# dash-robotics/perception

Measured on AMD Instinct MI355X. Metric: frames/sec (640x480 D435 cloud, plane+cluster+ICP), higher is better.
Workload: dtype f32

## Files before the change

### perception_amd/csrc/k_icp_lat.hip

```cpp
#include "kernels.hpp"
#include "icp_solve.hpp"

namespace cd {

struct LatFaces {
    int nface;
    unsigned m0[LAT_MAX_FACES], m1[LAT_MAX_FACES], m2[LAT_MAX_FACES];
    float c[LAT_MAX_FACES];
    int nx, ny, nz, tox, toy, toz;
    float ox, oy, oz, ivx, ivy, ivz;
};

template <int THREADS>
__device__ __forceinline__ void lat_stage(const IcpLattice* __restrict__ L, LatFaces& F, float4* s_tab, int4* s_face) {
    F.nface = L->nface;
#pragma unroll
    for (int f = 0; f < LAT_MAX_FACES; ++f) { F.m0[f] = L->m0[f]; F.m1[f] = L->m1[f]; F.m2[f] = L->m2[f]; F.c[f] = L->c[f]; }
    F.nx = L->n[0]; F.ny = L->n[1]; F.nz = L->n[2]; F.tox = L->toff[0]; F.toy = L->toff[1]; F.toz = L->toff[2];
    F.ox = L->noi[0]; F.oy = L->noi[1]; F.oz = L->noi[2]; F.ivx = L->inv[0]; F.ivy = L->inv[1]; F.ivz = L->inv[2];
    for (int i = threadIdx.x; i < L->ntab; i += THREADS) s_tab[i] = L->tab[i];
    if (threadIdx.x < LAT_MAX_FACES) {
        const int f = threadIdx.x, w = L->w[f], u = L->fast[f], v = 3 - w - u;
        s_face[f] = make_int4(w, u, L->base[f], __float_as_int(L->c[f]));
        s_face[LAT_MAX_FACES + f] = make_int4(L->toff[u], L->toff[v < 0 || v > 2 ? 0 : v], L->n[u], 0);
    }
    __syncthreads();
}

__device__ __forceinline__ float lat_pick(unsigned m, float a, float b) {
    float r;
    asm("v_bfi_b32 %0, %1, %2, %3" : "=v"(r) : "s"(m), "v"(a), "v"(b));
    return r;
}

__device__ __forceinline__ void lat_axis(const float4* s_tab, int toff, int n, float o_inv_neg, float inv, float q, float& f, int& ig_out, bool& lo_out,
                                         bool& hi_out, float& t, float& gap) {
    int ig;
    {
        const float pos = __builtin_fmaf(q, inv, o_inv_neg);
        asm("v_cvt_rpi_i32_f32 %0, %1" : "=v"(ig) : "v"(pos));
    }
    ig = min(max(ig, 0), n - 1);
    const float4 W = s_tab[toff + ig];
    const float d0 = __fsub_rn(q, W.x), d1 = __fsub_rn(q, W.y), d2 = __fsub_rn(q, W.z);
    const float f0 = __fmul_rn(d0, d0), f1 = __fmul_rn(d1, d1), f2 = __fmul_rn(d2, d2);
    const float g_mid = __fsub_rn(f0, f1), g_hi = __fsub_rn(f1, f2);
    const bool lo = f0 < f1;
    const bool hi = f2 < f1;
    f = f1; t = W.y; gap = g_mid;
    f = lo ? f0 : f; t = lo ? W.x : t; gap = lo ? 0.f : gap;
    f = hi ? f2 : f; t = hi ? W.z : t; gap = hi ? g_hi : gap;
    ig_out = ig; lo_out = lo; hi_out = hi;
}

__device__ __forceinline__ float lat_sum(float ax, float ay, float az) { return __fadd_rn(__fadd_rn(ax, ay), az); }

struct LatHit {
    float d;
    float nx, ny, nz;
    int face;
    int ix, iy, iz;
};

template <bool TIES, int NF>
__device__ __forceinline__ LatHit lat_nearest(const float4* s_tab, const int4* s_face, const LatFaces& F, float qx, float qy, float qz) {
    float fx, fy, fz, tx, ty, tz, gx, gy, gz;
    int cx, cy, cz;
    bool lox, hix, loy, hiy, loz, hiz;
    LatHit h;
    lat_axis(s_tab, F.tox, F.nx, F.ox, F.ivx, qx, fx, cx, lox, hix, tx, gx);
    lat_axis(s_tab, F.toy, F.ny, F.oy, F.ivy, qy, fy, cy, loy, hiy, ty, gy);
    lat_axis(s_tab, F.toz, F.nz, F.oz, F.ivz, qz, fz, cz, loz, hiz, tz, gz);
    h.ix = h.iy = h.iz = 0;
    h.d = __uint_as_float(0x7f800000u); h.face = 0;
#pragma unroll
    for (int f = 0; f < NF; ++f) {
        const unsigned m0 = F.m0[f], m1 = F.m1[f], m2 = F.m2[f];
        const float dc = __fsub_rn(lat_pick(m0, qx, lat_pick(m1, qy, qz)), F.c[f]);
        const float fc = __fmul_rn(dc, dc);
        const float d = lat_sum(lat_pick(m0, fc, fx), lat_pick(m1, fc, fy), lat_pick(m2, fc, fz));
        const bool better = d < h.d;
        h.d = better ? d : h.d;
        if (TIES) h.face = better ? f : h.face;
    }
    h.nx = tx; h.ny = ty; h.nz = tz;
    if (TIES) {
        const int4 fd = s_face[h.face];
        const float c = __int_as_float(fd.w);
        h.nx = fd.x == 0 ? c : tx; h.ny = fd.x == 1 ? c : ty; h.nz = fd.x == 2 ? c : tz;
        const float gsel = fd.x == 0 ? fminf(gy, gz) : (fd.x == 1 ? fminf(gx, gz) : fminf(gx, gy));
        const bool maybe = gsel <= __fmul_rn(h.d, 4.76837158203125e-07f);
        if (ballot64(maybe)) {
            h.ix = cx + (hix ? 1 : 0) - (lox ? 1 : 0); h.iy = cy + (hiy ? 1 : 0) - (loy ? 1 : 0); h.iz = cz + (hiz ? 1 : 0) - (loz ? 1 : 0);
            for (int f = 0; f < F.nface; ++f) {
                const bool mine = maybe && h.face == f;
                if (!ballot64(mine)) continue;
                const int4 gd = s_face[f];
                const int w = __builtin_amdgcn_readfirstlane(gd.x), u = __builtin_amdgcn_readfirstlane(gd.y), v = 3 - w - u;
                const float cc = __int_as_float(__builtin_amdgcn_readfirstlane(gd.w));
                const int4 ge = s_face[LAT_MAX_FACES + f];
                const int toff_u = __builtin_amdgcn_readfirstlane(ge.x), toff_v = __builtin_amdgcn_readfirstlane(ge.y);
                const float qw = w == 0 ? qx : (w == 1 ? qy : qz), qu = u == 0 ? qx : (u == 1 ? qy : qz), qv = v == 0 ? qx : (v == 1 ? qy : qz);
                const float dc = __fsub_rn(qw, cc);
                const float fc = __fmul_rn(dc, dc);
                float fu = u == 0 ? fx : (u == 1 ? fy : fz), fv = v == 0 ? fx : (v == 1 ? fy : fz);
                float tu = u == 0 ? tx : (u == 1 ? ty : tz), tv = v == 0 ? tx : (v == 1 ? ty : tz);
                int iu = u == 0 ? h.ix : (u == 1 ? h.iy : h.iz), iv = v == 0 ? h.ix : (v == 1 ? h.iy : h.iz);
                auto d_of = [&](float a_u, float a_v) {
                    const float ax = w == 0 ? fc : (u == 0 ? a_u : a_v), ay = w == 1 ? fc : (u == 1 ? a_u : a_v), az = w == 2 ? fc : (u == 2 ? a_u : a_v);
                    return lat_sum(ax, ay, az);
                };
                for (;;) {
                    const int j = max(iv - 1, 0);
                    const float t = s_tab[toff_v + j].y;
                    const float dd = __fsub_rn(qv, t);
                    const float a = __fmul_rn(dd, dd);
                    const bool go = mine && iv > 0 && d_of(fu, a) == h.d;
                    iv = go ? j : iv; fv = go ? a : fv; tv = go ? t : tv;
                    if (!ballot64(go)) break;
                }
                for (;;) {
                    const int i = max(iu - 1, 0);
                    const float t = s_tab[toff_u + i].y;
                    const float dd = __fsub_rn(qu, t);
                    const float a = __fmul_rn(dd, dd);
                    const bool go = mine && iu > 0 && d_of(a, fv) == h.d;
                    iu = go ? i : iu; fu = go ? a : fu; tu = go ? t : tu;
                    if (!ballot64(go)) break;
                }
                const bool ux = mine && u == 0, uy = mine && u == 1, uz = mine && u == 2, vx = mine && v == 0, vy = mine && v == 1, vz = mine && v == 2;
                h.ix = ux ? iu : (vx ? iv : h.ix); h.nx = ux ? tu : (vx ? tv : h.nx);
                h.iy = uy ? iu : (vy ? iv : h.iy); h.ny = uy ? tu : (vy ? tv : h.ny);
                h.iz = uz ? iu : (vz ? iv : h.iz); h.nz = uz ? tu : (vz ? tv : h.nz);
            }
        }
    }
    return h;
}

__device__ __forceinline__ int lat_index(const int4* s_face, const LatFaces& F, const LatHit& h) {
    const int4 fd = s_face[h.face];
    const int w = fd.x, u = fd.y, v = 3 - w - u;
    const int iu = u == 0 ? h.ix : (u == 1 ? h.iy : h.iz), iv = v == 0 ? h.ix : (v == 1 ? h.iy : h.iz);
    return fd.z + iv * s_face[LAT_MAX_FACES + h.face].z + iu;
}

__device__ __forceinline__ int lat_solve(IcpState* so, const unsigned long long* A, int n, const IcpParams& prm) {
    float Tn[16];
    umeyama_from_moments(A, n, Tn);
    float Tf[16];
    for (int i = 0; i < 4; ++i)
        for (int j = 0; j < 4; ++j)
            Tf[4 * i + j] = ((Tn[4 * i] * so->Tfinal[j] + Tn[4 * i + 1] * so->Tfinal[4 + j]) + Tn[4 * i + 2] * so->Tfinal[8 + j]) +
                            Tn[4 * i + 3] * so->Tfinal[12 + j];
    for (int i = 0; i < 16; ++i) so->Tfinal[i] = Tf[i];
    so->iters += 1;
    int done = 0;
    if (so->iters >= prm.max_iter) {
        done = 1;
    } else {
        const double cos_angle = 0.5 * (double)(((Tn[0] + Tn[5]) + Tn[10]) - 1.0f);
        const double translation_sqr = (double)((Tn[3] * Tn[3] + Tn[7] * Tn[7]) + Tn[11] * Tn[11]);
        if (cos_angle >= prm.rot_thr && translation_sqr <= prm.trans_eps) {
            done = 1;
        } else {
            const double mse = unfix(A[15], FIX_SHIFT_D2) / (double)n;
            if (fabs(mse - so->prev_mse) < prm.abs_mse) done = 1;
            else if (fabs(mse - so->prev_mse) / so->prev_mse < prm.rel_mse) done = 1;
            so->prev_mse = mse;
        }
    }
    for (int i = 0; i < 16; ++i) so->T[i] = Tn[i];
    return done;
}

#ifdef CD_LAT_TIMERS
__device__ unsigned long long g_lat_stats[8];
extern "C" int cd_debug_lat_stats(unsigned long long* out, int reset) {
    if (hipMemcpyFromSymbol(out, HIP_SYMBOL(g_lat_stats), sizeof(g_lat_stats)) != hipSuccess) return -1;
    if (reset) { unsigned long long z[8] = {0}; (void)hipMemcpyToSymbol(HIP_SYMBOL(g_lat_stats), z, sizeof(z)); }
    return 0;
}
#define LAT_T(k) { const long long tn_ = clock64(); tph[k] += tn_ - tlast; tlast = tn_; }
#else
#define LAT_T(k)
#endif

template <int SHIFT>
struct LatFix {
    static constexpr unsigned long long C = ((unsigned long long)(1023 + 52 - SHIFT) << 52) | (1ull << 51);
    static __device__ __forceinline__ unsigned long long bits(float v) {
        return (unsigned long long)__double_as_longlong(__dadd_rn((double)v, __longlong_as_double((long long)C)));
    }
};
static_assert(LatFix<32>::C == 0x4138000000000000ull && LatFix<36>::C == 0x40f8000000000000ull, "constants of lat_fix");
static_assert(FIX_SHIFT == 32 && FIX_SHIFT_D2 == 36, "k_icp_lat's moment sums are written for these scales");

struct LatSlot {
    int k, src_off, n, tslot;
    int phase;
    int gen;
    int ready;
    int pad;
};
enum { LAT_ITER = 0, LAT_FIT = 1, LAT_EMPTY = 2 };

#ifndef CD_LAT_WAVES_PER_EU
#define CD_LAT_WAVES_PER_EU 4
#endif
template <int CPW, int WPC>
__global__ void __launch_bounds__(CPW * WPC * WAVE, CD_LAT_WAVES_PER_EU)
k_icp_lat(int nitems, const int* __restrict__ order, const IcpCluster* __restrict__ cl, IcpState* __restrict__ st,
          unsigned long long* __restrict__ accf, const IcpLattice* __restrict__ lats, float4* __restrict__ src,
          const float4* __restrict__ src0, int* __restrict__ queue, unsigned long long* __restrict__ busy,
          unsigned long long* __restrict__ busy_out, IcpParams prm) {
    __shared__ float4 s_tab[CPW][LAT_MAX_TAB];
    __shared__ int4 s_face[CPW][2 * LAT_MAX_FACES];
    __shared__ unsigned long long s_acc[CPW][16];
    __shared__ IcpState s_so[CPW];
    __shared__ LatSlot s_slot[CPW];
    __shared__ int s_flags[2];
    const int lane = threadIdx.x & 63, wave = threadIdx.x >> 6;
    const int slot = wave / WPC, sub = wave % WPC;
    const long long wg_t0 = wall_clock64();
    auto refill = [&](int s) {
        LatSlot& sl = s_slot[s];
        for (int i = 0; i < 16; ++i) s_acc[s][i] = 0ull;
        sl.ready = 0;
        for (;;) {
            const int item = atomicAdd(queue, 1);
            if (item >= nitems) { sl.phase = LAT_EMPTY; return; }
            const int k = order[item];
            if (st[2 * (size_t)k].done) continue;
            const IcpCluster c = cl[k];
            sl.k = k; sl.src_off = c.src_off; sl.n = c.n; sl.tslot = c.slot;
            s_so[s] = st[2 * (size_t)k];
            sl.phase = LAT_ITER;
            sl.gen += 1;
            return;
        }
    };
    if (threadIdx.x < CPW) { s_slot[threadIdx.x].gen = 0; refill(threadIdx.x); }
    if (threadIdx.x == 0) { s_flags[0] = 0; s_flags[1] = 1; }
    __syncthreads();
    int my_gen = 0;
#ifdef CD_LAT_TIMERS
    long long tph[6] = {0, 0, 0, 0, 0, 0}, tlast = clock64();
#endif
    for (;;) {
        if (s_flags[1]) {
            const LatSlot sl = s_slot[slot];
            const bool mine = sl.phase != LAT_EMPTY && sl.gen != my_gen;
            if (mine) {
                const IcpLattice* __restrict__ L = lats + sl.tslot;
                for (int i = sub * WAVE + lane; i < L->ntab; i += WPC * WAVE) s_tab[slot][i] = L->tab[i];
                if (sub == 0 && lane < LAT_MAX_FACES) {
                    const int f = lane, w = L->w[f], u = L->fast[f], v = 3 - w - u;
                    s_face[slot][f] = make_int4(w, u, L->base[f], __float_as_int(L->c[f]));
                    s_face[slot][LAT_MAX_FACES + f] = make_int4(L->toff[u], L->toff[v < 0 || v > 2 ? 0 : v], L->n[u], 0);
                }
                my_gen = sl.gen;
            }
            __syncthreads();
        }
        LAT_T(5)
        {
            const int phase = __builtin_amdgcn_readfirstlane(s_slot[slot].phase), n = __builtin_amdgcn_readfirstlane(s_slot[slot].n);
            const int src_off = __builtin_amdgcn_readfirstlane(s_slot[slot].src_off), tslot = __builtin_amdgcn_readfirstlane(s_slot[slot].tslot);
            const int npass = (n + 63) >> 6;
            float4* pts = src + src_off;
            const float4* tab = s_tab[slot];
            const int4* face = s_face[slot];
            LatFaces F;
            {
                const IcpLattice* __restrict__ L = lats + (phase == LAT_EMPTY ? 0 : tslot);
                F.nface = L->nface;
#pragma unroll
                for (int f = 0; f < LAT_MAX_FACES; ++f) { F.m0[f] = L->m0[f]; F.m1[f] = L->m1[f]; F.m2[f] = L->m2[f]; F.c[f] = L->c[f]; }
                F.nx = L->n[0]; F.ny = L->n[1]; F.nz = L->n[2]; F.tox = L->toff[0]; F.toy = L->toff[1]; F.toz = L->toff[2];
                F.ox = L->noi[0]; F.oy = L->noi[1]; F.oz = L->noi[2]; F.ivx = L->inv[0]; F.ivy = L->inv[1]; F.ivz = L->inv[2];
            }
            const bool nf3 = F.nface <= 3;
            if (phase == LAT_ITER) {
                const bool moved = s_so[slot].iters > 0;
                float T[12];
#pragma unroll
                for (int i = 0; i < 12; ++i) T[i] = s_so[slot].T[i];
                unsigned long long S[16];
#pragma unroll
                for (int i = 0; i < 16; ++i) S[i] = 0ull;
                float4 pnext = pts[min((sub << 6) + lane, n - 1)];
                for (int pss = sub; pss < npass; pss += WPC) {
                    const int myq = (pss << 6) + lane;
                    const bool act = myq < n;
                    const float4 p = pnext;
                    pnext = pts[min(((pss + WPC) << 6) + lane, n - 1)];
                    float px = p.x, py = p.y, pz = p.z;
                    if (moved) {
                        xform(T, p.x, p.y, p.z, px, py, pz);
                        if (act) pts[myq] = make_float4(px, py, pz, p.w);
                    }
                    const LatHit h = nf3 ? lat_nearest<true, 3>(tab, face, F, px, py, pz) : lat_nearest<true, LAT_MAX_FACES>(tab, face, F, px, py, pz);
                    if (act) {
                        const float pv[3] = {px, py, pz}, qv[3] = {h.nx, h.ny, h.nz};
                        const float big_c = fmaxf(fmaxf(fmaxf(fabsf(px), fabsf(py)), fabsf(pz)), fmaxf(fmaxf(fabsf(h.nx), fabsf(h.ny)), fabsf(h.nz)));
                        if (big_c < 256.f && h.d < 16384.f) {
#pragma unroll
                            for (int a = 0; a < 3; ++a) {
                                S[a] += LatFix<FIX_SHIFT>::bits(pv[a]);
                                S[3 + a] += LatFix<FIX_SHIFT>::bits(qv[a]);
#pragma unroll
                                for (int b = 0; b < 3; ++b) S[6 + 3 * a + b] += LatFix<FIX_SHIFT>::bits(__fmul_rn(qv[a], pv[b]));
                            }
                            S[15] += LatFix<FIX_SHIFT_D2>::bits(h.d);
                        } else {
#pragma unroll
                            for (int a = 0; a < 3; ++a) {
                                S[a] += (unsigned long long)fixq(pv[a], FIX_SHIFT) + LatFix<FIX_SHIFT>::C;
                                S[3 + a] += (unsigned long long)fixq(qv[a], FIX_SHIFT) + LatFix<FIX_SHIFT>::C;
#pragma unroll
                                for (int b = 0; b < 3; ++b) S[6 + 3 * a + b] += (unsigned long long)fixq(__fmul_rn(qv[a], pv[b]), FIX_SHIFT) + LatFix<FIX_SHIFT>::C;
                            }
                            S[15] += (unsigned long long)fixq(h.d, FIX_SHIFT_D2) + LatFix<FIX_SHIFT_D2>::C;
                        }
                    }
                }
                if (sub < npass) wave_fold_to_lds(S, 16, s_acc[slot]);
                if (sub == 0 && lane == 0) s_slot[slot].ready = 1;
            } else if (phase == LAT_FIT) {
                const float4* pts0 = src0 + src_off;
                float T[12], Tf[12];
#pragma unroll
                for (int i = 0; i < 12; ++i) {
                    T[i] = __int_as_float(__builtin_amdgcn_readfirstlane(__float_as_int(s_so[slot].T[i])));
                    Tf[i] = __int_as_float(__builtin_amdgcn_readfirstlane(__float_as_int(s_so[slot].Tfinal[i])));
                }
                unsigned long long S[16];
#pragma unroll
                for (int i = 0; i < 16; ++i) S[i] = 0ull;
                float4 pnext = pts[min((sub << 6) + lane, n - 1)], p0next = pts0[min((sub << 6) + lane, n - 1)];
                for (int pss = sub; pss < npass; pss += WPC) {
                    const int myq = (pss << 6) + lane;
                    const bool act = myq < n;
                    const float4 p = pnext, p0 = p0next;
                    pnext = pts[min(((pss + WPC) << 6) + lane, n - 1)];
                    p0next = pts0[min(((pss + WPC) << 6) + lane, n - 1)];
                    float ox, oy, oz;
                    xform(T, p.x, p.y, p.z, ox, oy, oz);
                    if (act) pts[myq] = make_float4(ox, oy, oz, p.w);
                    float qx, qy, qz;
                    xform(Tf, p0.x, p0.y, p0.z, qx, qy, qz);
                    const LatHit h = nf3 ? lat_nearest<false, 3>(tab, face, F, qx, qy, qz) : lat_nearest<false, LAT_MAX_FACES>(tab, face, F, qx, qy, qz);
                    if (act) S[0] += h.d < 16384.f ? LatFix<FIX_SHIFT_D2>::bits(h.d) : (unsigned long long)fixq(h.d, FIX_SHIFT_D2) + LatFix<FIX_SHIFT_D2>::C;
                }
                if (sub < npass) wave_fold_to_lds(S, 1, s_acc[slot]);
            }
        }
        LAT_T(0)
        __syncthreads();
        LAT_T(1)
        if (threadIdx.x == 0) s_flags[1] = 0;
        if (threadIdx.x < CPW) {
            const int s = threadIdx.x;
            LatSlot& sl = s_slot[s];
            const unsigned long long off = (unsigned long long)sl.n * LatFix<FIX_SHIFT>::C, off_d = (unsigned long long)sl.n * LatFix<FIX_SHIFT_D2>::C;
            if (sl.phase == LAT_ITER && sl.ready) {
                for (int i = 0; i < 15; ++i) s_acc[s][i] -= off;
                s_acc[s][15] -= off_d;
                if (lat_solve(&s_so[s], s_acc[s], sl.n, prm)) sl.phase = LAT_FIT;
                for (int i = 0; i < 16; ++i) s_acc[s][i] = 0ull;
                sl.ready = 0;
            } else if (sl.phase == LAT_FIT) {
                s_so[s].done = 1;
                s_so[s].converged = 1;
                st[2 * (size_t)sl.k] = s_so[s];
                st[2 * (size_t)sl.k + 1] = s_so[s];
                accf[sl.k] = s_acc[s][0] - off_d;
                refill(s);
                if (sl.phase != LAT_EMPTY) s_flags[1] = 1;
            }
        }
        if (threadIdx.x == 0) {
            int all_empty = 1;
            for (int s = 0; s < CPW; ++s) all_empty &= s_slot[s].phase == LAT_EMPTY ? 1 : 0;
            s_flags[0] = all_empty;
        }
        LAT_T(2)
        __syncthreads();
        LAT_T(3)
#ifdef CD_LAT_TIMERS
        tph[4] += 1;
#endif
        if (s_flags[0]) break;
    }
#ifdef CD_LAT_TIMERS
    if (threadIdx.x == 0) for (int i = 0; i < 6; ++i) atomicAdd(&g_lat_stats[i], (unsigned long long)tph[i]);
#endif
    if (threadIdx.x == 0 && busy) {
        atomicAdd(busy, (unsigned long long)(wall_clock64() - wg_t0) * (unsigned long long)(CPW * WPC));
        if (busy_out) {
            __threadfence();
            if (atomicAdd(queue + 1, 1) == (int)gridDim.x - 1) {
                __threadfence();
                *busy_out = atomicAdd(busy, 0ull);
            }
        }
    }
}

__global__ void __launch_bounds__(BLOCK) k_lat_nn(const IcpLattice* __restrict__ L, const float4* __restrict__ q, int n, int* __restrict__ out_idx,
                                                  float* __restrict__ out_d2) {
    __shared__ float4 s_tab[LAT_MAX_TAB];
    __shared__ int4 s_face[2 * LAT_MAX_FACES];
    LatFaces F;
    lat_stage<BLOCK>(L, F, s_tab, s_face);
    for (int base = blockIdx.x * BLOCK; base < n; base += gridDim.x * BLOCK) {
        const int i = base + threadIdx.x;
        const float4 p = q[i < n ? i : n - 1];
        const LatHit h = lat_nearest<true, LAT_MAX_FACES>(s_tab, s_face, F, p.x, p.y, p.z);
        const LatHit g = lat_nearest<false, 3>(s_tab, s_face, F, p.x, p.y, p.z);
        if (i < n) { out_idx[i] = lat_index(s_face, F, h); out_d2[i] = (F.nface > 3 || h.d == g.d) ? h.d : __uint_as_float(0x7fc00000u); }
    }
}

template <int CPW, int WPC>
static void launch_lat_shape(hipStream_t s, int nitems, int n_wg, const int* order, const IcpCluster* cl, IcpState* st, unsigned long long* accf,
                             const IcpLattice* lats, float4* src, const float4* src0, int* queue, unsigned long long* busy, unsigned long long* busy_out,
                             IcpParams prm) {
    hipLaunchKernelGGL((k_icp_lat<CPW, WPC>), dim3(n_wg), dim3(CPW * WPC * WAVE), 0, s, nitems, order, cl, st, accf, lats, src, src0, queue, busy, busy_out, prm);
}
void launch_icp_lat(hipStream_t s, int nitems, int cpw, int wpc, int n_wg, const int* order, const IcpCluster* cl, IcpState* st,
                    unsigned long long* accf, const IcpLattice* lats, float4* src, const float4* src0, int* queue, unsigned long long* busy,
                    unsigned long long* busy_out, IcpParams prm) {
    if (nitems <= 0 || n_wg <= 0) return;
#define CD_LAT_CASE(C, W) if (cpw == C && wpc == W) return launch_lat_shape<C, W>(s, nitems, n_wg, order, cl, st, accf, lats, src, src0, queue, busy, busy_out, prm);
    CD_LAT_CASE(1, 1) CD_LAT_CASE(1, 2) CD_LAT_CASE(1, 4) CD_LAT_CASE(1, 8) CD_LAT_CASE(1, 16)
    CD_LAT_CASE(2, 1) CD_LAT_CASE(2, 2) CD_LAT_CASE(2, 4)
    CD_LAT_CASE(4, 1) CD_LAT_CASE(4, 2) CD_LAT_CASE(4, 4)
    CD_LAT_CASE(8, 1) CD_LAT_CASE(8, 2)
#undef CD_LAT_CASE
    launch_lat_shape<1, 4>(s, nitems, n_wg, order, cl, st, accf, lats, src, src0, queue, busy, busy_out, prm);
}
void launch_lat_nn(hipStream_t s, const IcpLattice* lat, const float4* q, int n, int* out_idx, float* out_d2) {
    if (n <= 0) return;
    const int g = (n + BLOCK - 1) / BLOCK;
    hipLaunchKernelGGL(k_lat_nn, dim3(g < 1024 ? g : 1024), dim3(BLOCK), 0, s, lat, q, n, out_idx, out_d2);
}

}
```

Measured before the change: 186,000.

## Parallelize per-cluster ICP Procrustes solve across a wavefront using lane reads and DPP

Replaces the single-thread-per-slot lat_solve in the persistent ICP lattice kernel with a wave-cooperative solver. Lanes load the 16 accumulators in parallel, build the covariance via readlane, run Jacobi SVD with U/V columns rotated across lanes using DPP shifts, and compose Tfinal per lane. The block-wide all-empty flag computation is replaced by each thread scanning the slot phases, and one shared flag is dropped. This is meant to shorten the serial solve phase that stalls all waves between barriers. In exchange it adds lane-shuffle code and wave-divergent control flow, and a debug kernel is included to compare it against the serial solver.

Measured after the change: 185,700, median of 6. Within noise of the previous version (-0.2%).

```diff
diff --git a/perception_amd/csrc/icp_solve_wave.hpp b/perception_amd/csrc/icp_solve_wave.hpp
--- /dev/null
+++ b/perception_amd/csrc/icp_solve_wave.hpp
@@ -0,0 +1,191 @@
+#pragma once
+#include "icp_solve.hpp"
+
+namespace cd {
+
+__device__ __forceinline__ float wv_read(float v, int l) { return __int_as_float(__builtin_amdgcn_readlane(__float_as_int(v), l)); }
+__device__ __forceinline__ double wv_read(double v, int l) {
+    const long long b = __double_as_longlong(v);
+    const unsigned lo = (unsigned)__builtin_amdgcn_readlane((int)(unsigned)b, l), hi = (unsigned)__builtin_amdgcn_readlane((int)(b >> 32), l);
+    return __longlong_as_double((long long)(((unsigned long long)hi << 32) | lo));
+}
+template <int D>
+__device__ __forceinline__ float wv_shift(float v) {
+    static_assert(D != 0 && D > -16 && D < 16, "DPP row shift");
+    return __int_as_float(__builtin_amdgcn_update_dpp(0, __float_as_int(v), D > 0 ? 0x100 + D : 0x110 - D, 0xf, 0xf, false));
+}
+
+template <int P, int Q>
+__device__ __forceinline__ float wv_rot_cols(float m, int col, bool is_v, const Rot& ju, const Rot& jv) {
+    const float from_q = wv_shift<-(P - Q)>(m), from_p = wv_shift<P - Q>(m);
+    const float c = is_v ? jv.c : ju.c, s = is_v ? jv.s : ju.s;
+    const bool at_p = col == P, at_q = col == Q;
+    const float r = __fadd_rn(__fmul_rn(c, m), __fmul_rn(at_p ? -s : s, at_p ? from_q : from_p));
+    return (at_p || at_q) ? r : m;
+}
+
+template <int P, int Q>
+__device__ __forceinline__ void wv_jacobi_pq(float W[3][3], float& uv, int col, bool is_v, bool& finished) {
+    const float precision = 2.0f * 1.1920928955078125e-07f;
+    const float consider_zero = 2.0f * 1.401298464324817e-45f;
+    const float thr = fmaxf(consider_zero, precision * fmaxf(fabsf(W[P][P]), fabsf(W[Q][Q])));
+    if (fabsf(W[P][Q]) > thr || fabsf(W[Q][P]) > thr) {
+        finished = false;
+        const float m00 = W[P][P], m01 = W[P][Q], m10 = W[Q][P], m11 = W[Q][Q];
+        Rot rot1;
+        const float t = m00 + m11, d = m10 - m01;
+        if (t == 0.f) {
+            rot1.c = 0.f;
+            rot1.s = d > 0.f ? 1.f : -1.f;
+        } else {
+            const float u = d / t;
+            rot1.c = 1.0f / sqrtf(1.0f + u * u);
+            rot1.s = rot1.c * u;
+        }
+        const float n00 = rot1.c * m00 + rot1.s * m10, n01 = rot1.c * m01 + rot1.s * m11;
+        const float n11 = -rot1.s * m01 + rot1.c * m11;
+        const Rot j_right = make_jacobi(n00, n01, n11);
+        const Rot j_left = rot_mul(rot1, rot_T(j_right));
+        apply_left(W, P, Q, j_left);
+        apply_right(W, P, Q, j_right);
+        uv = wv_rot_cols<P, Q>(uv, col, is_v, rot_T(j_left), j_right);
+    }
+}
+
+__device__ inline int lat_solve_wave(IcpState* so, unsigned long long* A, unsigned long long off, unsigned long long off_d, int n,
+                                     const IcpParams& prm) {
+    const int lane = threadIdx.x & 63;
+    const int k16 = lane & 15, ti = k16 >> 2, tj = k16 & 3;
+    const unsigned long long raw = A[k16];
+    const float tf0 = so->Tfinal[tj], tf1 = so->Tfinal[4 + tj], tf2 = so->Tfinal[8 + tj], tf3 = so->Tfinal[12 + tj];
+    const int iters = so->iters + 1;
+    const double prev_mse = so->prev_mse;
+    const double v = unfix(raw - (k16 == 15 ? off_d : off), k16 == 15 ? FIX_SHIFT_D2 : FIX_SHIFT) / (double)n;
+    const double mp0 = wv_read(v, 0), mp1 = wv_read(v, 1), mp2 = wv_read(v, 2), mq0 = wv_read(v, 3), mq1 = wv_read(v, 4), mq2 = wv_read(v, 5);
+    const double mse = wv_read(v, 15);
+    const int sa = k16 < 9 ? 0 : (k16 < 12 ? 1 : 2), sb = (k16 - 6) - 3 * sa;
+    const float sig = (float)(v - (sa == 0 ? mq0 : (sa == 1 ? mq1 : mq2)) * (sb == 0 ? mp0 : (sb == 1 ? mp1 : mp2)));
+    float sigma[3][3];
+#pragma unroll
+    for (int a = 0; a < 3; ++a)
+#pragma unroll
+        for (int b = 0; b < 3; ++b) sigma[a][b] = wv_read(sig, 6 + 3 * a + b);
+    float scale = 0.f;
+#pragma unroll
+    for (int i = 0; i < 3; ++i)
+#pragma unroll
+        for (int j = 0; j < 3; ++j) scale = fmaxf(scale, fabsf(sigma[i][j]));
+    if (scale == 0.f) scale = 1.f;
+    const float wl = sig / scale;
+    float W[3][3];
+#pragma unroll
+    for (int i = 0; i < 3; ++i)
+#pragma unroll
+        for (int j = 0; j < 3; ++j) W[i][j] = wv_read(wl, 6 + 3 * i + j);
+    const bool is_v = lane >= 16;
+    const int e = lane & 15, row = e < 3 ? 0 : (e < 6 ? 1 : 2), col = e - 3 * row;
+    float uv = row == col ? 1.f : 0.f;
+    bool finished = false;
+    for (int sweep = 0; sweep < 64 && !finished; ++sweep) {
+        finished = true;
+        wv_jacobi_pq<1, 0>(W, uv, col, is_v, finished);
+        wv_jacobi_pq<2, 0>(W, uv, col, is_v, finished);
+        wv_jacobi_pq<2, 1>(W, uv, col, is_v, finished);
+    }
+    float S[3];
+#pragma unroll
+    for (int i = 0; i < 3; ++i) S[i] = fabsf(W[i][i]);
+    {
+        const float wd = col == 0 ? W[0][0] : (col == 1 ? W[1][1] : W[2][2]);
+        const float a = fabsf(wd);
+        const float f = wd / a;
+        if (!is_v && a != 0.f) uv *= f;
+    }
+    float U[3][3], V[3][3];
+#pragma unroll
+    for (int r = 0; r < 3; ++r)
+#pragma unroll
+        for (int c = 0; c < 3; ++c) { U[r][c] = wv_read(uv, 3 * r + c); V[r][c] = wv_read(uv, 16 + 3 * r + c); }
+#define CD_SWAP_COLS(a, b)                                                  \
+    {                                                                       \
+        float t_ = S[a]; S[a] = S[b]; S[b] = t_;                            \
+        _Pragma("unroll") for (int r = 0; r < 3; ++r) {                     \
+            t_ = U[r][a]; U[r][a] = U[r][b]; U[r][b] = t_;                  \
+            t_ = V[r][a]; V[r][a] = V[r][b]; V[r][b] = t_;                  \
+        }                                                                   \
+    }
+    {
+        int pos = 0;
+        float mxv = S[0];
+        if (S[1] > mxv) { mxv = S[1]; pos = 1; }
+        if (S[2] > mxv) { mxv = S[2]; pos = 2; }
+        if (mxv != 0.f) {
+            if (pos == 1) CD_SWAP_COLS(0, 1)
+            else if (pos == 2) CD_SWAP_COLS(0, 2)
+            if (S[2] > S[1]) CD_SWAP_COLS(1, 2)
+        }
+    }
+#undef CD_SWAP_COLS
+#pragma unroll
+    for (int i = 0; i < 3; ++i) S[i] *= scale;
+    float sd[3] = {1.f, 1.f, 1.f};
+    if (det3(sigma) < 0.f) sd[2] = -1.f;
+    int rank = 0;
+#pragma unroll
+    for (int i = 0; i < 3; ++i)
+        if (!(fabsf(S[i]) <= fabsf(S[0]) * 1e-5f)) ++rank;
+    if (rank == 2) {
+        sd[0] = 1.f; sd[1] = 1.f;
+        sd[2] = (det3(U) * det3(V) > 0.f) ? 1.f : -1.f;
+    }
+    float R[3][3];
+#pragma unroll
+    for (int i = 0; i < 3; ++i)
+#pragma unroll
+        for (int j = 0; j < 3; ++j)
+            R[i][j] = ((U[i][0] * sd[0]) * V[j][0] + (U[i][1] * sd[1]) * V[j][1]) + (U[i][2] * sd[2]) * V[j][2];
+    const float mpf[3] = {(float)mp0, (float)mp1, (float)mp2};
+    const float mqf[3] = {(float)mq0, (float)mq1, (float)mq2};
+    float Tn[16];
+#pragma unroll
+    for (int i = 0; i < 3; ++i) {
+#pragma unroll
+        for (int j = 0; j < 3; ++j) Tn[4 * i + j] = R[i][j];
+        Tn[4 * i + 3] = mqf[i] - ((R[i][0] * mpf[0] + R[i][1] * mpf[1]) + R[i][2] * mpf[2]);
+    }
+    Tn[12] = Tn[13] = Tn[14] = 0.f;
+    Tn[15] = 1.f;
+    const float r0 = ti == 0 ? Tn[0] : (ti == 1 ? Tn[4] : (ti == 2 ? Tn[8] : Tn[12]));
+    const float r1 = ti == 0 ? Tn[1] : (ti == 1 ? Tn[5] : (ti == 2 ? Tn[9] : Tn[13]));
+    const float r2 = ti == 0 ? Tn[2] : (ti == 1 ? Tn[6] : (ti == 2 ? Tn[10] : Tn[14]));
+    const float r3 = ti == 0 ? Tn[3] : (ti == 1 ? Tn[7] : (ti == 2 ? Tn[11] : Tn[15]));
+    const float tf = ((r0 * tf0 + r1 * tf1) + r2 * tf2) + r3 * tf3;
+    int done = 0;
+    double new_prev = prev_mse;
+    if (iters >= prm.max_iter) {
+        done = 1;
+    } else {
+        const double cos_angle = 0.5 * (double)(((Tn[0] + Tn[5]) + Tn[10]) - 1.0f);
+        const double translation_sqr = (double)((Tn[3] * Tn[3] + Tn[7] * Tn[7]) + Tn[11] * Tn[11]);
+        if (cos_angle >= prm.rot_thr && translation_sqr <= prm.trans_eps) {
+            done = 1;
+        } else {
+            if (fabs(mse - prev_mse) < prm.abs_mse) done = 1;
+            else if (fabs(mse - prev_mse) / prev_mse < prm.rel_mse) done = 1;
+            new_prev = mse;
+        }
+    }
+    if (lane < 16) {
+        so->Tfinal[lane] = tf;
+        A[lane] = 0ull;
+    }
+    if (lane == 0) {
+#pragma unroll
+        for (int i = 0; i < 16; ++i) so->T[i] = Tn[i];
+        so->iters = iters;
+        so->prev_mse = new_prev;
+    }
+    return done;
+}
+
+}
diff --git a/perception_amd/csrc/k_icp_lat.hip b/perception_amd/csrc/k_icp_lat.hip
--- a/perception_amd/csrc/k_icp_lat.hip
+++ b/perception_amd/csrc/k_icp_lat.hip
@@ -1,5 +1,6 @@
 #include "kernels.hpp"
 #include "icp_solve.hpp"
+#include "icp_solve_wave.hpp"
 
 namespace cd {
 
@@ -219,7 +220,7 @@
     __shared__ unsigned long long s_acc[CPW][16];
     __shared__ IcpState s_so[CPW];
     __shared__ LatSlot s_slot[CPW];
-    __shared__ int s_flags[2];
+    __shared__ int s_refilled;
     const int lane = threadIdx.x & 63, wave = threadIdx.x >> 6;
     const int slot = wave / WPC, sub = wave % WPC;
     const long long wg_t0 = wall_clock64();
@@ -241,14 +242,14 @@
         }
     };
     if (threadIdx.x < CPW) { s_slot[threadIdx.x].gen = 0; refill(threadIdx.x); }
-    if (threadIdx.x == 0) { s_flags[0] = 0; s_flags[1] = 1; }
+    if (threadIdx.x == 0) s_refilled = 1;
     __syncthreads();
     int my_gen = 0;
 #ifdef CD_LAT_TIMERS
     long long tph[6] = {0, 0, 0, 0, 0, 0}, tlast = clock64();
 #endif
     for (;;) {
-        if (s_flags[1]) {
+        if (s_refilled) {
             const LatSlot sl = s_slot[slot];
             const bool mine = sl.phase != LAT_EMPTY && sl.gen != my_gen;
             if (mine) {
@@ -264,6 +265,7 @@
             __syncthreads();
         }
         LAT_T(5)
+        if (threadIdx.x == 0) s_refilled = 0;
         {
             const int phase = __builtin_amdgcn_readfirstlane(s_slot[slot].phase), n = __builtin_amdgcn_readfirstlane(s_slot[slot].n);
             const int src_off = __builtin_amdgcn_readfirstlane(s_slot[slot].src_off), tslot = __builtin_amdgcn_readfirstlane(s_slot[slot].tslot);
@@ -359,31 +361,26 @@
         LAT_T(0)
         __syncthreads();
         LAT_T(1)
-        if (threadIdx.x == 0) s_flags[1] = 0;
-        if (threadIdx.x < CPW) {
-            const int s = threadIdx.x;
-            LatSlot& sl = s_slot[s];
-            const unsigned long long off = (unsigned long long)sl.n * LatFix<FIX_SHIFT>::C, off_d = (unsigned long long)sl.n * LatFix<FIX_SHIFT_D2>::C;
-            if (sl.phase == LAT_ITER && sl.ready) {
-                for (int i = 0; i < 15; ++i) s_acc[s][i] -= off;
-                s_acc[s][15] -= off_d;
-                if (lat_solve(&s_so[s], s_acc[s], sl.n, prm)) sl.phase = LAT_FIT;
-                for (int i = 0; i < 16; ++i) s_acc[s][i] = 0ull;
-                sl.ready = 0;
-            } else if (sl.phase == LAT_FIT) {
-                s_so[s].done = 1;
-                s_so[s].converged = 1;
-                st[2 * (size_t)sl.k] = s_so[s];
-                st[2 * (size_t)sl.k + 1] = s_so[s];
-                accf[sl.k] = s_acc[s][0] - off_d;
-                refill(s);
-                if (sl.phase != LAT_EMPTY) s_flags[1] = 1;
+        if (sub == 0) {
+            LatSlot& sl = s_slot[slot];
+            const int phase = __builtin_amdgcn_readfirstlane(sl.phase), ready = __builtin_amdgcn_readfirstlane(sl.ready);
+            const int n = __builtin_amdgcn_readfirstlane(sl.n);
+            const unsigned long long off = (unsigned long long)n * LatFix<FIX_SHIFT>::C, off_d = (unsigned long long)n * LatFix<FIX_SHIFT_D2>::C;
+            if (phase == LAT_ITER && ready) {
+                const int done = lat_solve_wave(&s_so[slot], s_acc[slot], off, off_d, n, prm);
+                if (lane == 0) {
+                    if (done) sl.phase = LAT_FIT;
+                    sl.ready = 0;
+                }
+            } else if (phase == LAT_FIT && lane == 0) {
+                s_so[slot].done = 1;
+                s_so[slot].converged = 1;
+                st[2 * (size_t)sl.k] = s_so[slot];
+                st[2 * (size_t)sl.k + 1] = s_so[slot];
+                accf[sl.k] = s_acc[slot][0] - off_d;
+                refill(slot);
+                if (sl.phase != LAT_EMPTY) s_refilled = 1;
             }
-        }
-        if (threadIdx.x == 0) {
-            int all_empty = 1;
-            for (int s = 0; s < CPW; ++s) all_empty &= s_slot[s].phase == LAT_EMPTY ? 1 : 0;
-            s_flags[0] = all_empty;
         }
         LAT_T(2)
         __syncthreads();
@@ -391,7 +388,10 @@
 #ifdef CD_LAT_TIMERS
         tph[4] += 1;
 #endif
-        if (s_flags[0]) break;
+        bool all_empty = true;
+#pragma unroll
+        for (int s = 0; s < CPW; ++s) all_empty = all_empty && s_slot[s].phase == LAT_EMPTY;
+        if (all_empty) break;
     }
 #ifdef CD_LAT_TIMERS
     if (threadIdx.x == 0) for (int i = 0; i < 6; ++i) atomicAdd(&g_lat_stats[i], (unsigned long long)tph[i]);
@@ -406,6 +406,63 @@
             }
         }
     }
+}
+
+__global__ void __launch_bounds__(WAVE) k_debug_lat_solve(int nitems, const unsigned long long* __restrict__ sums, const int* __restrict__ ns,
+                                                          const IcpState* __restrict__ st_in, IcpParams prm, IcpState* __restrict__ out_serial,
+                                                          IcpState* __restrict__ out_wave, int* __restrict__ done_out) {
+    __shared__ unsigned long long s_acc[2][16];
+    __shared__ IcpState s_so[2];
+    const int i = blockIdx.x, lane = threadIdx.x;
+    if (i >= nitems) return;
+    const int n = ns[i];
+    const unsigned long long off = (unsigned long long)n * LatFix<FIX_SHIFT>::C, off_d = (unsigned long long)n * LatFix<FIX_SHIFT_D2>::C;
+    if (lane < 16) {
+        const unsigned long long r = sums[16 * (size_t)i + lane] + (lane == 15 ? off_d : off);
+        s_acc[0][lane] = r;
+        s_acc[1][lane] = r;
+    }
+    if (lane < 2) s_so[lane] = st_in[i];
+    __syncthreads();
+    if (lane == 0) {
+        for (int k = 0; k < 15; ++k) s_acc[0][k] -= off;
+        s_acc[0][15] -= off_d;
+        done_out[2 * (size_t)i] = lat_solve(&s_so[0], s_acc[0], n, prm);
+    }
+    __syncthreads();
+    const int dw = lat_solve_wave(&s_so[1], s_acc[1], off, off_d, n, prm);
+    if (lane == 0) done_out[2 * (size_t)i + 1] = dw;
+    __syncthreads();
+    if (lane == 0) {
+        out_serial[i] = s_so[0];
+        out_wave[i] = s_so[1];
+        for (int k = 0; k < 16; ++k) done_out[2 * (size_t)nitems + 16 * (size_t)i + k] = s_acc[1][k] != 0ull;
+    }
+}
+extern "C" int cd_debug_lat_solve(int nitems, const unsigned long long* sums, const int* ns, const IcpState* st_in, const IcpParams* prm,
+                                  IcpState* out_serial, IcpState* out_wave, int* done_out) {
+    if (nitems <= 0 || !sums || !ns || !st_in || !prm || !out_serial || !out_wave || !done_out) return (int)hipErrorInvalidValue;
+    const size_t nsum = sizeof(unsigned long long) * 16 * (size_t)nitems, nst = sizeof(IcpState) * (size_t)nitems, nd = sizeof(int) * 18 * (size_t)nitems;
+    unsigned long long* d_sums = nullptr;
+    int *d_ns = nullptr, *d_done = nullptr;
+    IcpState *d_in = nullptr, *d_ser = nullptr, *d_wave = nullptr;
+    hipError_t e = hipSuccess;
+    auto step = [&](hipError_t r) { if (e == hipSuccess) e = r; };
+    step(hipMalloc(&d_sums, nsum)); step(hipMalloc(&d_ns, sizeof(int) * (size_t)nitems)); step(hipMalloc(&d_done, nd));
+    step(hipMalloc(&d_in, nst)); step(hipMalloc(&d_ser, nst)); step(hipMalloc(&d_wave, nst));
+    step(hipMemcpy(d_sums, sums, nsum, hipMemcpyHostToDevice));
+    step(hipMemcpy(d_ns, ns, sizeof(int) * (size_t)nitems, hipMemcpyHostToDevice));
+    step(hipMemcpy(d_in, st_in, nst, hipMemcpyHostToDevice));
+    if (e == hipSuccess) {
+        hipLaunchKernelGGL(k_debug_lat_solve, dim3(nitems), dim3(WAVE), 0, 0, nitems, d_sums, d_ns, d_in, *prm, d_ser, d_wave, d_done);
+        step(hipGetLastError());
+        step(hipDeviceSynchronize());
+    }
+    step(hipMemcpy(out_serial, d_ser, nst, hipMemcpyDeviceToHost));
+    step(hipMemcpy(out_wave, d_wave, nst, hipMemcpyDeviceToHost));
+    step(hipMemcpy(done_out, d_done, nd, hipMemcpyDeviceToHost));
+    (void)hipFree(d_sums); (void)hipFree(d_ns); (void)hipFree(d_done); (void)hipFree(d_in); (void)hipFree(d_ser); (void)hipFree(d_wave);
+    return (int)e;
 }
 
 __global__ void __launch_bounds__(BLOCK) k_lat_nn(const IcpLattice* __restrict__ L, const float4* __restrict__ q, int n, int* __restrict__ out_idx,
```
